# assafmu/wav2letter_pytorch

Hardware: AMD Instinct MI355X
Metric: audio-frames/sec/GPU (fwd+bwd+CTC), Wav2Letter 64-mel x 1000-frame bf16 (higher is better)
Workload: dtype bf16

## Files before the change

wav2letter_pytorch_amd/csrc/conv_igemm.hip:

```cpp
#include "common.h"
#include "../../include/w2l_hip.h"
#include <algorithm>
#include <array>
#include <map>
#include <vector>
#include <mutex>
#include <tuple>
#include <type_traits>
#include <utility>

namespace {

constexpr int BK = 64;
constexpr int ROWB = BK * 2;

struct IgemmParams {
    const bf16_raw* x;
    const bf16_raw* w;
    void* y;
    const float* bias;
    union { float* stats; uint8_t* fz_q; };
    int stats_slots;
    int64_t x_rows_per_utt;
    int64_t x_max_row;
    int N, Cin, Cout, Tout, Kw, stride, dil;
    int tiles_t, ncols, xrows_lds;
    int y_f32, accumulate;
    int splits;
    float* slabs;
    unsigned* tickets;
    int sk_ranges, sk_total;
    float descale;
    union { const float* descale_dev; unsigned long long* fz_clip; };
    union { const bf16_raw* bn_y; const bf16_raw* fz_res; };
    union { const float* bn_scale; const float* fz_scale; };
    union { const float* bn_shift; const float* fz_shift; };
    union { const float* bn_mean; const bf16_raw* fz_res_lo; };
    union { const float* bn_invstd; bf16_raw* fz_out; };
    union { const uint8_t* bn_mask; bf16_raw* fz_out_lo; };
    union { const int32_t* bn_lens; const int32_t* fz_lens; };
    union { int bn_T; int fz_rows; };
    union { int bn_pad_l; int fz_pad_l; };
    union { int bn_pad_mode; int fz_pad_mode; };
    union { int bn_per; int fz_pad_r; };
    int bn_Tp;
    union { int bn_act; int fz_act; };
    union { float bn_gk; float fz_qscale; };
};

typedef int v4i __attribute__((ext_vector_type(4)));
typedef int v8i __attribute__((ext_vector_type(8)));
__device__ __forceinline__ f32x4 mfma_e4m3_k128(bf16x8 a_lo, bf16x8 a_hi, bf16x8 b_lo, bf16x8 b_hi, f32x4 c) {
    const v4i al = __builtin_bit_cast(v4i, a_lo), ah = __builtin_bit_cast(v4i, a_hi);
    const v4i bl = __builtin_bit_cast(v4i, b_lo), bh = __builtin_bit_cast(v4i, b_hi);
    const v8i av = __builtin_shufflevector(al, ah, 0, 1, 2, 3, 4, 5, 6, 7);
    const v8i bv = __builtin_shufflevector(bl, bh, 0, 1, 2, 3, 4, 5, 6, 7);
    return __builtin_amdgcn_mfma_scale_f32_16x16x128_f8f6f4(av, bv, c, 0, 0, 0, 0x7f7f7f7f, 0, 0x7f7f7f7f);
}

__device__ __forceinline__ void glds16(const void* gsrc, void* lds_dst_wave_base) {
    __builtin_amdgcn_global_load_lds((const __attribute__((address_space(1))) void*)gsrc,
                                     (__attribute__((address_space(3))) void*)lds_dst_wave_base, 16, 0, 0);
}

template <int G> struct QVec { typedef unsigned type __attribute__((ext_vector_type(G))); };
template <> struct QVec<1> { typedef unsigned type; };

struct SkPiece { int tile, s_begin, s_end, nsplit, split; int64_t slab_base; };
__host__ __device__ inline SkPiece sk_piece(int W, int G, int S_, int r, int w_cur, int w_end) {
    SkPiece q;
    q.tile = w_cur / S_;
    q.s_begin = w_cur - q.tile * S_;
    q.s_end = q.s_begin + (w_end - w_cur) < S_ ? q.s_begin + (w_end - w_cur) : S_;
    const int r_lo = (int)((((int64_t)q.tile * S_ + 1) * G + W - 1) / W) - 1;
    const int r_hi = (int)((((int64_t)q.tile * S_ + S_) * G + W - 1) / W) - 1;
    q.nsplit = r_hi - r_lo + 1;
    q.split = r - r_lo;
    q.slab_base = (int64_t)r_lo + q.tile;
    return q;
}

template <int MW, int NW, int MS, int NS, int S, int PIPE, bool F8 = false, int EPI = 0, bool SK = false>
__global__ __launch_bounds__(64 * MW * NW, 2) void conv_igemm_kernel(IgemmParams p) {
    static_assert(!SK || (!F8 && EPI == 0 && S == 1), "stream-K is built for the plain bf16 stride-1 kernels");
    static_assert(!(F8 && PIPE != 0), "the e4m3 kernel is built for K-loop structure 0 only");
    static_assert(EPI != 1 || (!F8 && S == 1), "the fused BatchNorm-backward epilogue belongs to bf16 data gradients");
    constexpr int ESZ = F8 ? 1 : 2;
    constexpr int BKE = ROWB / ESZ;
    constexpr int BM = 16 * MW * MS, BN = 16 * NW * NS, NWAVES = MW * NW, NT = 64 * NWAVES;
    extern __shared__ __attribute__((aligned(1024))) char smem[];
    const int tid = threadIdx.x;
    const int lane = tid & 63;
    const int wave = __builtin_amdgcn_readfirstlane(tid >> 6);
    const int wm = wave / NW, wn = wave % NW;

    const int lin = xcd_remap(blockIdx.x, gridDim.x);
    int w_cur = 0, w_end = 0;
    if constexpr (SK) {
        w_cur = (int)(((int64_t)p.sk_total * lin) / p.sk_ranges);
        w_end = (int)(((int64_t)p.sk_total * (lin + 1)) / p.sk_ranges);
    }
    do {
    int split, tile, nsplit, sk_begin = 0, sk_end = 0;
    int64_t slab_base;
    if constexpr (SK) {
        __syncthreads();
        const SkPiece q = sk_piece(p.sk_total, p.sk_ranges, (p.Cin / (ROWB / (F8 ? 1 : 2))) * p.Kw, lin, w_cur, w_end);
        tile = q.tile;
        sk_begin = q.s_begin;
        sk_end = q.s_end;
        w_cur += sk_end - sk_begin;
        nsplit = q.nsplit;
        split = q.split;
        slab_base = q.slab_base;
    } else {
        nsplit = p.splits;
        split = nsplit > 1 ? lin % nsplit : 0;
        tile = nsplit > 1 ? lin / nsplit : lin;
        slab_base = (int64_t)tile * nsplit;
    }
    const int tm = tile / p.ncols;
    const int col = tile - tm * p.ncols;
    const int n = col / p.tiles_t;
    const int tt = col - n * p.tiles_t;
    const int m0 = tm * BM;
    const int t0 = tt * BN;

    constexpr int s = S;
    const int d = p.dil, Kw = p.Kw, Cin = p.Cin;
    const int xrows = p.xrows_lds;
    char* wbuf0 = smem;
    char* wbuf1 = smem + BM * ROWB;
    char* xbuf0 = smem + 2 * BM * ROWB;
    char* xbuf1 = xbuf0 + xrows * ROWB;

    const int64_t xrow0 = (int64_t)n * p.x_rows_per_utt + (int64_t)t0 * s;

    const int srow = lane >> 3;
    const int schunk = lane & 7;
    const int gchunk = schunk ^ srow;
    constexpr int WGROUPS = BM / 8;
    constexpr int W_PER_WAVE = (WGROUPS + NWAVES - 1) / NWAVES;
    unsigned w_voff[W_PER_WAVE];
#pragma unroll
    for (int i = 0; i < W_PER_WAVE; ++i) {
        int co = m0 + (wave + i * NWAVES) * 8 + srow;
        co = co < p.Cout ? co : p.Cout - 1;
        w_voff[i] = (unsigned)co * (unsigned)Cin * (unsigned)ESZ + (unsigned)gchunk * 16u;
    }
    const int64_t w_tap_bytes = (int64_t)p.Cout * Cin * ESZ;
    auto stage_w = [&](char* dst, int kw, int c) {
        W2L_DIAG_SKIP_DMA(p);
        const char* slab = reinterpret_cast<const char*>(p.w) + kw * w_tap_bytes + c * (BK * 2);
#pragma unroll
        for (int i = 0; i < W_PER_WAVE; ++i) {
            const int grp = wave + i * NWAVES;
            if ((WGROUPS % NWAVES == 0) || grp < WGROUPS) glds16(slab + w_voff[i], dst + grp * 1024);
        }
    };
    auto stage_x = [&](char* dst, int c) {
        W2L_DIAG_SKIP_DMA(p);
        const int ngrp = xrows >> 3;
        for (int grp = wave; grp < ngrp; grp += NWAVES) {
            int64_t r = xrow0 + grp * 8 + srow;
            r = r < p.x_max_row ? r : p.x_max_row;
            const char* src = reinterpret_cast<const char*>(p.x) + (r * Cin + (int64_t)c * BKE) * ESZ + gchunk * 16;
            glds16(src, dst + grp * 1024);
        }
    };

    f32x4 acc[MS][NS];
#pragma unroll
    for (int i = 0; i < MS; ++i)
#pragma unroll
        for (int j = 0; j < NS; ++j) acc[i][j] = f32x4{0.f, 0.f, 0.f, 0.f};

    const int nchunks = Cin / BKE;
    const int total_steps = nchunks * Kw;
    const int s_begin = SK ? sk_begin : (nsplit > 1 ? (int)(((int64_t)total_steps * split) / nsplit) : 0);
    const int s_end = SK ? sk_end : (nsplit > 1 ? (int)(((int64_t)total_steps * (split + 1)) / nsplit) : total_steps);
    const int nsteps = s_end - s_begin;
    const int c_first = s_begin / Kw, kw_first = s_begin - c_first * Kw;

    const int fr = lane & 15, fq = lane >> 4;
    constexpr int CH1_XOR = F8 ? 16 : 64;
    const int ch0 = F8 ? 2 * fq : fq;
    const int a_lane0 = (wm * MS * 16 + fr) * ROWB + ((ch0 ^ (fr & 7)) << 4);
    const int a_lane1 = a_lane0 ^ CH1_XOR;
    const int b_row0 = (wn * NS * 16 + fr) * s;

    if constexpr (PIPE == 0) {
        stage_x((c_first & 1) ? xbuf1 : xbuf0, c_first);
        stage_w(wbuf0, kw_first, c_first);

        int kw = kw_first, c = c_first;
        for (int step = 0; step < nsteps; ++step) {
            asm volatile("s_waitcnt vmcnt(0)" ::: "memory");
            __syncthreads();
            int kw_n = kw + 1, c_n = c;
            if (kw_n == Kw) { kw_n = 0; c_n = c + 1; }
            if (step + 1 < nsteps) {
                stage_w((step & 1) ? wbuf0 : wbuf1, kw_n, c_n);
                if (kw_n == 0) stage_x((c_n & 1) ? xbuf1 : xbuf0, c_n);
            }
            const char* wb = (step & 1) ? wbuf1 : wbuf0;
            const char* xb = (c & 1) ? xbuf1 : xbuf0;
            const char* A0 = wb + a_lane0;
            const char* A1 = wb + a_lane1;
            const int tsh = b_row0 + kw * d;
            const int sw0 = ((ch0 ^ (tsh & 7)) << 4);
            const char* Bb = xb + (tsh << 7);
            const char* B0 = Bb + sw0;
            const char* B1 = Bb + (sw0 ^ CH1_XOR);
            bf16x8 a0[MS], b0[NS], a1[MS], b1[NS];
    #pragma unroll
// ... 189 lines not shown
                    const bool ok = co_ok[g] && t < Tout;
                    f32x4 v = acc[mi0 + g][ni] * descale + bias4[g];
                    v = v * sc4[g] + sh4[g];
                    if (p.fz_res && ok) {
                        const u16x4 rv = *reinterpret_cast<const u16x4*>(p.fz_res + ((int64_t)n * Tout + t) * Cout + co);
#pragma unroll
                        for (int r = 0; r < 4; ++r) v[r] += bf16_bits_to_f32(rv[r]);
                    }
                    u16x4 hi;
                    float a[4];
#pragma unroll
                    for (int r = 0; r < 4; ++r) {
                        a[r] = v[r];
                        if (p.fz_act == 1) a[r] = fminf(fmaxf(a[r], 0.f), 20.f);
                        else if (p.fz_act == 2) a[r] = fmaxf(a[r], 0.f);
                        if (t >= len_n) a[r] = 0.f;
                        hi[r] = f32_to_bf16_bits(a[r]);
                        if (ok && fabsf(a[r]) > q_limit) ++clipped;
                        a[r] = fminf(fmaxf(a[r] * qs, -448.f), 448.f);
                    }
                    int w = __builtin_amdgcn_cvt_pk_fp8_f32(a[0], a[1], 0, false);
                    w = __builtin_amdgcn_cvt_pk_fp8_f32(a[2], a[3], w, true);
                    q[g] = (unsigned)w;
                    if (obase && ok) {
                        put(pl + t, co, hi);
                        if (p.fz_pad_mode == 1) {
                            if (t >= 1 && t <= pl) put(pl - t, co, hi);
                            const int j = Tout - 1 - t;
                            if (j >= 1 && j <= pr) put(pl + Tout - 1 + j, co, hi);
                        }
                    }
                    if (obase && p.fz_pad_mode != 1 && tt == 0 && co_ok[g]) {
                        const u16x4 z = u16x4{0, 0, 0, 0};
                        if (tl < pl) put(tl, co, z);
                        if (tl < pr) put(pl + Tout + tl, co, z);
                    }
                }
#pragma unroll
                for (int b = 1; b < G; b <<= 1) {
                    const bool up = (fq & b) != 0;
#pragma unroll
                    for (int i = 0; i < G; ++i) {
                        if (i & b) continue;
                        const unsigned send = up ? q[i] : q[i | b];
                        const unsigned recv = (unsigned)__shfl_xor((int)send, 16 * b, 64);
                        if (up) q[i] = recv; else q[i | b] = recv;
                    }
                }
                if (qbase) {
                    qvec qv = {}, z = {};
                    if constexpr (G == 1) {
                        qv = q[0];
                    } else {
#pragma unroll
                        for (int g = 0; g < G; ++g) qv[g] = q[g];
                    }
                    if (coq_ok && t < Tout) {
                        putq(pl + t, qv);
                        if (p.fz_pad_mode == 1) {
                            if (t >= 1 && t <= pl) putq(pl - t, qv);
                            const int j = Tout - 1 - t;
                            if (j >= 1 && j <= pr) putq(pl + Tout - 1 + j, qv);
                        }
                    }
                    if (p.fz_pad_mode != 1 && tt == 0 && coq_ok) {
                        if (tl < pl) putq(tl, z);
                        if (tl < pr) putq(pl + Tout + tl, z);
                    }
                }
            }
        };
#pragma unroll
        for (int g4 = 0; g4 < MS / 4; ++g4) group(std::integral_constant<int, 4>{}, g4 * 4);
        if constexpr ((MS & 3) >= 2) group(std::integral_constant<int, 2>{}, (MS / 4) * 4);
        if constexpr (MS & 1) group(std::integral_constant<int, 1>{}, MS - 1);
        if (p.fz_clip) {
#pragma unroll
            for (int m = 1; m < 64; m <<= 1) clipped += __shfl_xor(clipped, m, 64);
            __syncthreads();
            unsigned* red = reinterpret_cast<unsigned*>(smem);
            if (lane == 0) red[wave] = clipped;
            __syncthreads();
            if (tid == 0) {
                unsigned total = 0;
                for (int w = 0; w < NWAVES; ++w) total += red[w];
                if (total) atomicAdd(p.fz_clip, (unsigned long long)total);
            }
        }
    } else if constexpr (EPI == 2) {
        const int pl = p.fz_pad_l, pr = p.fz_pad_r;
        const int len_n = p.fz_lens ? p.fz_lens[n] : Tout;
        bf16_raw* const obase = p.fz_out + (int64_t)n * p.fz_rows * Cout;
        bf16_raw* const obase_lo = p.fz_out_lo ? p.fz_out_lo + (int64_t)n * p.fz_rows * Cout : nullptr;
        auto put = [&](int row, int co, u16x4 hi, u16x4 lo) {
            const int64_t o = (int64_t)row * Cout + co;
            *reinterpret_cast<u16x4*>(obase + o) = hi;
            if (obase_lo) *reinterpret_cast<u16x4*>(obase_lo + o) = lo;
        };
#pragma unroll
        for (int mi = 0; mi < MS; ++mi) {
            const int co = m0 + (wm * MS + mi) * 16 + fq * 4;
            const bool co_ok = co < Cout;
            f32x4 bias4 = f32x4{0.f, 0.f, 0.f, 0.f}, sc4 = f32x4{1.f, 1.f, 1.f, 1.f}, sh4 = bias4;
            if (p.bias && co_ok) bias4 = *reinterpret_cast<const f32x4*>(p.bias + co);
            if (p.fz_scale && co_ok) {
                sc4 = *reinterpret_cast<const f32x4*>(p.fz_scale + co);
                sh4 = *reinterpret_cast<const f32x4*>(p.fz_shift + co);
            }
#pragma unroll
            for (int ni = 0; ni < NS; ++ni) {
                const int tl = (wn * NS + ni) * 16 + fr;
                const int t = t0 + tl;
                const bool ok = co_ok && t < Tout;
                if (ok) {
                    const int64_t off = ((int64_t)n * Tout + t) * Cout + co;
                    f32x4 v = acc[mi][ni] + bias4;
                    if (p.accumulate) v += *reinterpret_cast<const f32x4*>(reinterpret_cast<const float*>(p.y) + off);
                    v = v * sc4 + sh4;
                    if (p.fz_res) {
                        const u16x4 rv = *reinterpret_cast<const u16x4*>(p.fz_res + off);
#pragma unroll
                        for (int r = 0; r < 4; ++r) v[r] += bf16_bits_to_f32(rv[r]);
                        if (p.fz_res_lo) {
                            const u16x4 rl = *reinterpret_cast<const u16x4*>(p.fz_res_lo + off);
#pragma unroll
                            for (int r = 0; r < 4; ++r) v[r] += bf16_bits_to_f32(rl[r]);
                        }
                    }
                    u16x4 hi, lo = u16x4{0, 0, 0, 0};
#pragma unroll
                    for (int r = 0; r < 4; ++r) {
                        float a = v[r];
                        if (p.fz_act == 1) a = fminf(fmaxf(a, 0.f), 20.f);
                        else if (p.fz_act == 2) a = fmaxf(a, 0.f);
                        if (t >= len_n) a = 0.f;
                        hi[r] = f32_to_bf16_bits(a);
                        if (obase_lo) lo[r] = f32_to_bf16_bits(a - bf16_bits_to_f32(hi[r]));
                    }
                    put(pl + t, co, hi, lo);
                    if (p.fz_pad_mode == 1) {
                        if (t >= 1 && t <= pl) put(pl - t, co, hi, lo);
                        const int j = Tout - 1 - t;
                        if (j >= 1 && j <= pr) put(pl + Tout - 1 + j, co, hi, lo);
                    }
                }
                if (p.fz_pad_mode != 1 && tt == 0 && co_ok) {
                    const u16x4 z = u16x4{0, 0, 0, 0};
                    if (tl < pl) put(tl, co, z, z);
                    if (tl < pr) put(pl + Tout + tl, co, z, z);
                }
            }
        }
    } else {
    float s1[MS][4], s2[MS][4];
#pragma unroll
    for (int mi = 0; mi < MS; ++mi) {
        const int co = m0 + (wm * MS + mi) * 16 + fq * 4;
        const bool co_ok = co < Cout;
        f32x4 bias4 = f32x4{0.f, 0.f, 0.f, 0.f};
        if (p.bias && co_ok) bias4 = *reinterpret_cast<const f32x4*>(p.bias + co);
#pragma unroll
        for (int r = 0; r < 4; ++r) { s1[mi][r] = 0.f; s2[mi][r] = 0.f; }
#pragma unroll
        for (int ni = 0; ni < NS; ++ni) {
            const int t = t0 + (wn * NS + ni) * 16 + fr;
            const bool ok = co_ok && t < Tout;
            f32x4 v = F8 ? acc[mi][ni] * descale + bias4 : acc[mi][ni] + bias4;
            const int64_t off = ((int64_t)n * Tout + t) * Cout + co;
            if (ok) {
                if (p.y_f32) {
                    float* yp = reinterpret_cast<float*>(p.y) + off;
                    if (p.accumulate) v += *reinterpret_cast<const f32x4*>(yp);
                    *reinterpret_cast<f32x4*>(yp) = v;
                } else {
                    u16x4 o;
#pragma unroll
                    for (int r = 0; r < 4; ++r) o[r] = f32_to_bf16_bits(v[r]);
                    *reinterpret_cast<u16x4*>(reinterpret_cast<bf16_raw*>(p.y) + off) = o;
                }
                if constexpr (EPI == 0) {
#pragma unroll
                    for (int r = 0; r < 4; ++r) { s1[mi][r] += v[r]; s2[mi][r] += v[r] * v[r]; }
                }
            }
        }
    }
    if constexpr (EPI == 1) {
        int64_t yrow[NS];
        bool live[NS];
#pragma unroll
        for (int ni = 0; ni < NS; ++ni) {
            const int t = t0 + (wn * NS + ni) * 16 + fr;
            const int tc = t < Tout ? t : Tout - 1;
            const int nu = (int)((unsigned)tc / (unsigned)p.bn_per);
            const int u = tc - nu * p.bn_per;
            int ts = u - p.bn_pad_l;
            bool lv = t < Tout && u < p.bn_Tp;
            if (ts < 0 || ts >= p.bn_T) {
                if (p.bn_pad_mode == 1) ts = ts < 0 ? -ts : 2 * (p.bn_T - 1) - ts;
                else lv = false;
            }
            ts = ts < 0 ? 0 : (ts >= p.bn_T ? p.bn_T - 1 : ts);
            if (lv && p.bn_lens && ts >= p.bn_lens[nu]) lv = false;
            live[ni] = lv;
            yrow[ni] = (int64_t)nu * p.bn_T + ts;
        }
        constexpr int CH = MS % 4 == 0 ? 4 : (MS % 2 == 0 ? 2 : 1);
        __syncthreads();
        float* red = reinterpret_cast<float*>(smem);
#pragma unroll
        for (int m0i = 0; m0i < MS; m0i += CH) {
            u16x4 yv[CH][NS];
            unsigned mb[CH][NS];
#pragma unroll
            for (int c = 0; c < CH; ++c) {
                int co = m0 + (wm * MS + m0i + c) * 16 + fq * 4;
                co = co < Cout ? co : Cout - 4;
#pragma unroll
                for (int ni = 0; ni < NS; ++ni) {
                    yv[c][ni] = *reinterpret_cast<const u16x4*>(p.bn_y + yrow[ni] * Cout + co);
                    mb[c][ni] = p.bn_mask ? (unsigned)p.bn_mask[yrow[ni] * (Cout >> 3) + (co >> 3)] : 0xFFu;
                }
            }
#pragma unroll
            for (int c = 0; c < CH; ++c) {
                const int mi = m0i + c;
                const int co = m0 + (wm * MS + mi) * 16 + fq * 4;
                const bool co_ok = co < Cout;
                const int cc = co_ok ? co : Cout - 4;
                f32x4 bsc = f32x4{1.f, 1.f, 1.f, 1.f}, bsh = f32x4{0.f, 0.f, 0.f, 0.f}, bmu = bsh, bis = bsh;
                if (p.bn_scale) { bsc = *reinterpret_cast<const f32x4*>(p.bn_scale + cc); bsh = *reinterpret_cast<const f32x4*>(p.bn_shift + cc); }
                if (p.bn_mean) { bmu = *reinterpret_cast<const f32x4*>(p.bn_mean + cc); bis = *reinterpret_cast<const f32x4*>(p.bn_invstd + cc); }
#pragma unroll
                for (int ni = 0; ni < NS; ++ni) {
                    const bool on = live[ni] && co_ok;
                    const unsigned bits = mb[c][ni] >> (co & 4);
#pragma unroll
                    for (int r = 0; r < 4; ++r) {
                        const float yf = bf16_bits_to_f32(yv[c][ni][r]);
                        const bool keep = (bits >> r) & 1u;
                        float z = yf * bsc[r] + bsh[r];
                        z = keep ? z * p.bn_gk : 0.f;
                        bool pass = keep && on;
                        if (p.bn_act == 1) pass = pass && z >= 0.f && z <= 20.f;
                        else if (p.bn_act == 2) pass = pass && z > 0.f;
                        const float g = pass ? acc[mi][ni][r] * p.bn_gk : 0.f;
                        s1[mi][r] += g;
                        s2[mi][r] += g * ((yf - bmu[r]) * bis[r]);
                    }
                }
#pragma unroll
                for (int r = 0; r < 4; ++r) {
                    float a = s1[mi][r], b = s2[mi][r];
#pragma unroll
                    for (int m = 1; m < 16; m <<= 1) {
                        a += __shfl_xor(a, m, 64);
                        b += __shfl_xor(b, m, 64);
                    }
                    if (fr == 0) {
                        const int cl = (wm * MS + mi) * 16 + fq * 4 + r;
                        red[(wn * 2 + 0) * BM + cl] = a;
                        red[(wn * 2 + 1) * BM + cl] = b;
                    }
                }
            }
        }
    }
    if (p.stats) {
        constexpr int HALVES = BN / 128;
        constexpr int WPH = NW / HALVES;
        static_assert(BN % 128 == 0 || true, "");
        float* red = reinterpret_cast<float*>(smem);
        if constexpr (EPI == 0) {
            __syncthreads();
#pragma unroll
            for (int mi = 0; mi < MS; ++mi)
#pragma unroll
                for (int r = 0; r < 4; ++r) {
                    float a = s1[mi][r], b = s2[mi][r];
#pragma unroll
                    for (int m = 1; m < 16; m <<= 1) {
                        a += __shfl_xor(a, m, 64);
                        b += __shfl_xor(b, m, 64);
                    }
                    if (fr == 0) {
                        const int cl = (wm * MS + mi) * 16 + fq * 4 + r;
                        red[(wn * 2 + 0) * BM + cl] = a;
                        red[(wn * 2 + 1) * BM + cl] = b;
                    }
                }
        }
        __syncthreads();
        if (p.stats_slots) {
            float* dst = p.stats + (((int64_t)n * p.tiles_t + tt) % p.stats_slots) * 2 * Cout;
            for (int cl = tid; cl < BM; cl += NT) {
                if (m0 + cl < Cout) {
                    float a = 0.f, b = 0.f;
#pragma unroll
                    for (int w = 0; w < NW; ++w) {
                        a += red[(w * 2 + 0) * BM + cl];
                        b += red[(w * 2 + 1) * BM + cl];
                    }
                    atomicAdd(dst + m0 + cl, a);
                    atomicAdd(dst + Cout + m0 + cl, b);
                }
            }
        } else {
        const int tiles128 = (Tout + 127) / 128;
        for (int idx = tid; idx < BM * HALVES; idx += NT) {
            const int h = idx / BM, cl = idx - h * BM;
            const int trow = tt * HALVES + h;
            if (m0 + cl < Cout && trow < tiles128) {
                float a = 0.f, b = 0.f;
#pragma unroll
                for (int w = 0; w < WPH; ++w) {
                    a += red[((h * WPH + w) * 2 + 0) * BM + cl];
                    b += red[((h * WPH + w) * 2 + 1) * BM + cl];
                }
                const int64_t srow = (int64_t)n * tiles128 + trow;
                float* dst = p.stats + srow * 2 * Cout;
                dst[m0 + cl] = a;
                dst[Cout + m0 + cl] = b;
            }
        }
        }
    }
    }
    } while (SK && w_cur < w_end);
}

struct TileCfg { int mw, nw, ms, ns; float eff; };
constexpr TileCfg kCfgs[] = {
    {2, 2, 2, 4, 0.83f}, {2, 2, 3, 4, 1.00f}, {2, 2, 4, 4, 1.00f}, {2, 2, 5, 4, 1.01f},
    {4, 2, 3, 4, 0.90f}, {4, 2, 4, 4, 0.92f},
    {2, 3, 2, 3, 0.80f}, {2, 3, 3, 3, 0.97f}, {2, 3, 4, 3, 0.97f}, {2, 3, 5, 3, 0.98f},
    {2, 4, 2, 4, 0.85f}, {2, 4, 3, 4, 0.97f}, {2, 4, 4, 4, 1.00f}, {2, 4, 5, 4, 1.04f},
    {2, 4, 6, 4, 1.10f}, {2, 4, 7, 4, 1.06f}, {2, 4, 8, 4, 1.12f},
    {2, 3, 4, 6, 1.00f}, {2, 3, 5, 6, 1.00f}, {2, 3, 6, 6, 1.00f}, {2, 3, 7, 6, 1.00f},
    {2, 4, 4, 6, 1.00f}, {2, 4, 5, 6, 1.00f}, {2, 4, 6, 6, 1.00f},
    {2, 4, 4, 7, 1.00f}, {2, 4, 5, 7, 1.00f},
};
constexpr int kNumCfgs = sizeof(kCfgs) / sizeof(kCfgs[0]);
constexpr int kSpillCfg = 20;

constexpr size_t kLdsBytes = 160 * 1024;
constexpr int kCUs = 256;
constexpr size_t kTicketBytes = 64 * 1024;
constexpr int kFzMaxPad = 96;
constexpr int kWaveCap = 16, kSkWaveCap = 8;

struct ConvProblem {
    const void* x;
    int64_t x_bstride, x_rows_total;
    const void* w;
    void* y;
    int y_f32, accumulate;
    const float* bias;
    float* stats;
    int N, Cin, Cout, Tout, Kw, stride, dil;
    void* ws;
    int64_t ws_bytes;
    hipStream_t stream;
    bool f8 = false;
    float descale = 1.f;
    const float* descale_dev = nullptr;
    int stats_slots = 0;
};

enum EpiKind { kEpiNone = 0, kEpiBnReduce, kEpiInfer, kEpiInferF8 };
struct Epilogue {
    EpiKind kind;
    struct { const w2l_bnact_t* d; int pad_l, pad_r, pad_mode, per; } bn;
    const w2l_bnact_epi_t* fz;
    void* out_q;
    float q_scale;
    int64_t* q_clipped;
};
constexpr Epilogue kNoEpilogue{};
static inline bool is_infer(const Epilogue* ep) { return ep->kind == kEpiInfer || ep->kind == kEpiInferF8; }

static int stats_flag(const ConvProblem& pr, const Epilogue* ep) {
    if (is_infer(ep)) return 3;
    return pr.stats == nullptr ? 0 : (!pr.f8 && pr.stats_slots > 0 ? 2 : 1);
}

struct TileGeom {
    int bm, bn, xrows, waves, tiles_m, tiles_t;
    size_t lds;
    int64_t blocks;
};
static TileGeom tile_geom(const TileCfg& c, const ConvProblem& pr) {
    TileGeom g;
    g.bm = 16 * c.mw * c.ms;
    g.bn = 16 * c.nw * c.ns;
    g.xrows = ((g.bn - 1) * pr.stride + (pr.Kw - 1) * pr.dil + 1 + 7) & ~7;
    g.waves = c.mw * c.nw;
    g.tiles_m = (pr.Cout + g.bm - 1) / g.bm;
    g.tiles_t = (pr.Tout + g.bn - 1) / g.bn;
    g.lds = 2 * (size_t)g.bm * ROWB + 2 * (size_t)g.xrows * ROWB;
    g.blocks = (int64_t)g.tiles_m * pr.N * g.tiles_t;
    return g;
}
static ConvProblem window_only(int Kw, int stride, int dil) {
    ConvProblem pr{};
    pr.Kw = Kw; pr.stride = stride; pr.dil = dil;
    return pr;
}
static int blocks_per_cu(const TileGeom& g, int wave_cap) {
    const int by_lds = (int)(kLdsBytes / g.lds), by_waves = wave_cap / g.waves;
    const int per_cu = by_lds < by_waves ? by_lds : by_waves;
    return per_cu < 1 ? 1 : per_cu;
}
static double last_round_fill(int64_t blocks, int64_t slots) {
// ... 65 lines not shown

template <int MW, int NW, int MS, int NS>
int launch_f8(const ConvPlan& pl) {
    if (pl.epi == 2) {
        if constexpr (f8_fused_built(NW, MS, NS)) {
            return launch_kernel(conv_igemm_kernel<MW, NW, MS, NS, 1, 0, true, 2>, pl);
        } else {
            w2l_set_error("conv1d_igemm_bnact_fp8: block shape not built for the fused epilogue");
            return 1;
        }
    }
    return launch_kernel(conv_igemm_kernel<MW, NW, MS, NS, 1, 0, true>, pl);
}

typedef int (*LaunchFn)(const ConvPlan&);
template <int I> constexpr LaunchFn kLaunchCfg = &launch_cfg<kCfgs[I].mw, kCfgs[I].nw, kCfgs[I].ms, kCfgs[I].ns>;
template <int I> constexpr LaunchFn kLaunchF8 = &launch_f8<kCfgs[I].mw, kCfgs[I].nw, kCfgs[I].ms, kCfgs[I].ns>;
template <size_t... I>
constexpr std::array<LaunchFn, sizeof...(I)> cfg_launchers(std::index_sequence<I...>) { return {{kLaunchCfg<(int)I>...}}; }
template <size_t... K>
constexpr std::array<LaunchFn, sizeof...(K)> f8_launchers(std::index_sequence<K...>) { return {{kLaunchF8<kF8Cfgs[K]>...}}; }
constexpr auto kCfgLaunchers = cfg_launchers(std::make_index_sequence<kNumCfgs>{});
constexpr auto kF8Launchers = f8_launchers(std::make_index_sequence<kNumF8Cfgs>{});

int launch(const ConvPlan& pl) { return (pl.f8 ? kF8Launchers[pl.idx] : kCfgLaunchers[pl.shape])(pl); }

}

constexpr int kSplits[] = {1, 2, 3, 4, 5, 6, 8, 0};
constexpr int kNumSplits = sizeof(kSplits) / sizeof(kSplits[0]);
constexpr int kMaxSplit = 8;
constexpr int kSkMinSteps = 8;
constexpr int kBaseCfgs = 2 * kNumCfgs;
static thread_local int g_force_cfg = -1;
static thread_local int g_force_f8 = -1;
static thread_local int g_stats_slots = 0;
extern "C" void w2l_conv_stats_mode(int slots) { g_stats_slots = slots < 0 ? 0 : (slots > 64 ? 64 : slots); }
extern "C" void w2l_conv_force_tile_config(int idx) { g_force_cfg = idx; }
extern "C" void w2l_conv_force_fp8_config(int idx) { g_force_f8 = idx; }
W2L_DIAG_IGEMM_EXPORTS

typedef std::tuple<int, int, int, int, int, int, int, int> ShapeKey;
static std::map<ShapeKey, int> g_tuned, g_tuned_f8;
static std::mutex g_tuned_mu;
static ShapeKey shape_key(const ConvProblem& pr, int sflag) {
    return ShapeKey(pr.N, pr.Cin, pr.Cout, pr.Tout, pr.Kw, pr.stride, pr.dil, sflag);
}

static bool cfg_feasible(int idx, const ConvProblem& pr, int sflag) {
    if (idx < 0 || idx >= kBaseCfgs * kNumSplits) return false;
    const int i = idx % kNumCfgs;
    const TileGeom g = tile_geom(kCfgs[i], pr);
    if (sflag == 1 && !bn128_ok(g)) return false;
    if (pr.stride != 1 && i != 2) return false;
    if (i == kSpillCfg) return false;
    return g.lds <= kLdsBytes;
}

static bool f8_feasible(int k, const ConvProblem& pr, int sflag) {
    if (k < 0 || k >= kNumF8Cfgs) return false;
    const TileCfg& c = kCfgs[kF8Cfgs[k]];
    const TileGeom g = tile_geom(c, pr);
    if (sflag == 3 && (!f8_fused_built(c.nw, c.ms, c.ns) || g.bn <= kFzMaxPad)) return false;
    if (sflag == 1 && !bn128_ok(g)) return false;
    return g.lds <= kLdsBytes;
}

static int choose_cfg(const ConvProblem& pr, int sflag, int forced) {
    if (forced >= 0) return (pr.f8 ? f8_feasible(forced, pr, sflag) : cfg_feasible(forced, pr, sflag)) ? forced : -1;
    {
        std::lock_guard<std::mutex> lock(g_tuned_mu);
        const auto& tuned = pr.f8 ? g_tuned_f8 : g_tuned;
        auto it = tuned.find(shape_key(pr, sflag));
        if (it != tuned.end()) return it->second;
    }
    int best = -1;
    double best_cost = 1e30;
    for (int k = 0; k < (pr.f8 ? kNumF8Cfgs : kNumCfgs); ++k) {
        if (!(pr.f8 ? f8_feasible(k, pr, sflag) : cfg_feasible(k, pr, sflag))) continue;
        const TileCfg& c = kCfgs[pr.f8 ? kF8Cfgs[k] : k];
        const double cost = tile_cost(tile_geom(c, pr), c.eff, pr.f8 ? 1.0 : 0.75, k);
        if (cost < best_cost) { best_cost = cost; best = k; }
    }
    return best;
}

extern "C" int w2l_conv_stat_tiles(int N, int Tout) { return N * ((Tout + 127) / 128); }

static size_t splitk_bytes(const TileGeom& g, int splits) {
    return kTicketBytes + (size_t)g.blocks * splits * g.bm * g.bn * sizeof(float);
}

static int sk_ranges(const TileGeom& g) { return kCUs * blocks_per_cu(g, kSkWaveCap); }

static bool sk_feasible(const TileGeom& g, const ConvProblem& pr) {
    if (pr.ws == nullptr || pr.stride != 1) return false;
    const int64_t tiles = g.blocks, steps = (int64_t)(pr.Cin / BK) * pr.Kw, G = sk_ranges(g);
    if (tiles * steps / G < kSkMinSteps || (tiles * steps + steps) * G >= (1LL << 31)) return false;
    return tiles * (int64_t)sizeof(unsigned) <= (int64_t)kTicketBytes &&
           (int64_t)kTicketBytes + (tiles + G) * g.bm * g.bn * (int64_t)sizeof(float) <= pr.ws_bytes;
}

static bool split_feasible(const TileGeom& g, int splits, const ConvProblem& pr) {
    if (splits == 1) return true;
    if (pr.ws == nullptr || (pr.Cin / BK) * pr.Kw < 2 * splits) return false;
    return (size_t)g.blocks * sizeof(unsigned) <= kTicketBytes && splitk_bytes(g, splits) <= (size_t)pr.ws_bytes;
}

static int check_infer_epi(const w2l_bnact_epi_t* e, int Tout, const char* who) {
    W2L_CHECK_ARG(e->pad_l >= 0 && e->pad_r >= 0 && e->pad_l <= kFzMaxPad && e->pad_r <= kFzMaxPad &&
                  e->out_rows >= e->pad_l + Tout + e->pad_r,
                  "%s: bad output geometry (pads %d,%d of at most %d; %d rows for %d frames)", who, e->pad_l, e->pad_r,
                  kFzMaxPad, e->out_rows, Tout);
    W2L_CHECK_ARG(e->pad_mode != 1 || (e->pad_l < Tout && e->pad_r < Tout), "%s: reflect pad (%d,%d) needs pad < T=%d", who,
                  e->pad_l, e->pad_r, Tout);
    W2L_CHECK_ARG((e->scale == nullptr) == (e->shift == nullptr) && e->act >= 0 && e->act <= 2 && (e->res || !e->res_lo),
                  "%s: scale/shift come together, act is 0..2, res_lo needs res", who);
    return 0;
}

static int plan(const ConvProblem& pr, const Epilogue* ep, int forced, ConvPlan& pl) {
    const char* who = pr.f8 ? "conv1d_igemm_fp8" : "conv1d_igemm";
    W2L_CHECK_ARG(pr.x && pr.w && (pr.y || is_infer(ep)), "%s: null pointer", who);
    W2L_CHECK_ARG(pr.f8 ? ep->kind == kEpiNone || ep->kind == kEpiInferF8 : ep->kind != kEpiInferF8,
                  "%s: epilogue of the other operand type", who);
    W2L_CHECK_ARG(pr.N > 0 && pr.Tout > 0 && pr.Kw > 0 && (pr.stride == 1 || (pr.stride == 2 && !pr.f8)) && pr.dil > 0,
                  "%s: bad sizes (stride must be 1 or 2; e4m3: 1)", who);
    const int cin_unit = pr.f8 ? 128 : 64;
    W2L_CHECK_ARG(pr.Cin % cin_unit == 0 && pr.Cin > 0, "%s: Cin=%d must be a positive multiple of %d", who, pr.Cin, cin_unit);
    W2L_CHECK_ARG(pr.Cout % 64 == 0 && pr.Cout > 0, "%s: Cout=%d must be a positive multiple of 64", who, pr.Cout);
    W2L_CHECK_ARG(pr.x_bstride % pr.Cin == 0, "%s: x_bstride must be a multiple of Cin", who);
    W2L_CHECK_ARG(!(pr.accumulate && !pr.y_f32), "%s: accumulate needs fp32 output", who);
    W2L_CHECK_ARG(pr.descale > 0.f, "%s: descale must be positive", who);
    IgemmParams& p = pl.p;
    p.x = (const bf16_raw*)pr.x;
    p.w = (const bf16_raw*)pr.w;
    p.y = pr.y;
    p.bias = pr.bias;
    p.stats = pr.stats;
    p.stats_slots = pr.stats ? pr.stats_slots : 0;
    p.x_rows_per_utt = pr.x_bstride / pr.Cin;
    p.x_max_row = pr.x_rows_total - 1;
    p.N = pr.N; p.Cin = pr.Cin; p.Cout = pr.Cout; p.Tout = pr.Tout; p.Kw = pr.Kw; p.stride = pr.stride; p.dil = pr.dil;
    p.y_f32 = pr.y_f32; p.accumulate = pr.accumulate;
    p.descale = pr.descale;
    p.descale_dev = pr.descale_dev;
    pl.epi = 0;
    if (ep->kind == kEpiBnReduce) {
        const w2l_bnact_t* d = ep->bn.d;
        const int pad_l = ep->bn.pad_l, pad_r = ep->bn.pad_r, per = ep->bn.per;
        W2L_CHECK_ARG(d && d->y && !d->y_f32 && !d->y2 && pr.stats && !pr.y_f32 && !pr.accumulate && !pr.bias && pr.N == 1 &&
                      pr.stride == 1,
                      "conv1d_dgrad_bnreduce: needs a bf16 single-branch layer, a statistics buffer and a flat bf16 output");
        W2L_CHECK_ARG(d->C == pr.Cout && per > 0 && pad_l >= 0 && pad_r >= 0 && (int64_t)d->N * per <= pr.Tout &&
                      per >= pad_l + d->T + pad_r,
                      "conv1d_dgrad_bnreduce: geometry mismatch (C=%d vs %d, per=%d, N=%d, rows=%d)", d->C, pr.Cout, per, d->N,
                      pr.Tout);
        W2L_CHECK_ARG(d->drop_p == 0.f || d->mask, "conv1d_dgrad_bnreduce: dropout needs the recorded mask");
        p.bn_y = (const bf16_raw*)d->y;
        p.bn_scale = d->scale; p.bn_shift = d->shift; p.bn_mean = d->mean; p.bn_invstd = d->invstd;
        p.bn_mask = d->drop_p > 0.f ? d->mask : nullptr;
        p.bn_lens = d->lens;
        p.bn_T = d->T; p.bn_pad_l = pad_l; p.bn_pad_mode = ep->bn.pad_mode; p.bn_per = per;
        p.bn_Tp = pad_l + d->T + pad_r;
        p.bn_act = d->act;
        p.bn_gk = d->drop_p > 0.f ? 1.f / (1.f - d->drop_p) : 1.f;
        pl.epi = 1;
    } else if (is_infer(ep)) {
        const w2l_bnact_epi_t* e = ep->fz;
        const bool q = ep->kind == kEpiInferF8 && ep->out_q != nullptr;
        const char* who_fz = pr.f8 ? "conv1d_igemm_bnact_fp8" : "conv1d_igemm_bnact";
        if (pr.f8) {
            W2L_CHECK_ARG(e && (e->out_hi || q) && !e->out_lo && !e->res_lo && !pr.y && !pr.stats && !pr.descale_dev,
                          "conv1d_igemm_bnact_fp8: needs an e4m3 or a bf16 output and takes no lo halves");
            W2L_CHECK_ARG(!q || (ep->q_scale > 0.f && ((uintptr_t)ep->out_q & 15) == 0),
                          "conv1d_igemm_bnact_fp8: the e4m3 output needs a positive scale and 16-byte alignment");
        } else {
            W2L_CHECK_ARG(e && pr.stats == nullptr && e->out_hi, "conv1d_igemm_bnact: null output / bad combination");
        }
        if (int rc = check_infer_epi(e, pr.Tout, who_fz)) return rc;
        p.stats_slots = 0;
        p.fz_q = q ? (uint8_t*)ep->out_q : nullptr;
        p.fz_qscale = q ? ep->q_scale : 1.f;
        p.fz_clip = q ? (unsigned long long*)ep->q_clipped : nullptr;
        p.fz_scale = e->scale; p.fz_shift = e->shift;
        p.fz_res = (const bf16_raw*)e->res; p.fz_res_lo = (const bf16_raw*)e->res_lo;
        p.fz_lens = e->lens;
        p.fz_out = (bf16_raw*)e->out_hi; p.fz_out_lo = (bf16_raw*)e->out_lo;
        p.fz_rows = e->out_rows; p.fz_pad_l = e->pad_l; p.fz_pad_r = e->pad_r; p.fz_pad_mode = e->pad_mode;
        p.fz_act = e->act;
        pl.epi = 2;
    }
    const int64_t need = (int64_t)(pr.N - 1) * p.x_rows_per_utt + (int64_t)(pr.Tout - 1) * pr.stride + (int64_t)(pr.Kw - 1) * pr.dil;
    W2L_CHECK_ARG(need <= p.x_max_row, "%s: padded input too small (need row %lld, have %lld)", who, (long long)need,
                  (long long)p.x_max_row);
    pl.idx = choose_cfg(pr, stats_flag(pr, ep), forced);
    W2L_CHECK_ARG(pl.idx >= 0, "%s: no block shape fits LDS (Kw=%d dil=%d stride=%d)", who, pr.Kw, pr.dil, pr.stride);
    pl.f8 = pr.f8;
    pl.shape = pr.f8 ? kF8Cfgs[pl.idx] : pl.idx % kNumCfgs;
    pl.pipe = pr.f8 ? 0 : (pl.idx % kBaseCfgs) / kNumCfgs;
    const TileCfg& c = kCfgs[pl.shape];
    const TileGeom g = tile_geom(c, pr);
    p.tiles_t = g.tiles_t;
    p.ncols = pr.N * g.tiles_t;
    p.xrows_lds = g.xrows;
    int splits = pr.f8 ? 1 : kSplits[pl.idx / kBaseCfgs];
    p.sk_ranges = 0;
    p.sk_total = 0;
    if (splits == 0) {
        if (pl.epi == 0 && sk_feasible(g, pr)) {
            p.sk_ranges = sk_ranges(g);
            p.sk_total = g.tiles_m * p.ncols * ((pr.Cin / BK) * pr.Kw);
        }
        splits = 1;
    }
    if (!split_feasible(g, splits, pr)) splits = 1;
    p.splits = splits;
    p.tickets = (unsigned*)pr.ws;
    p.slabs = pr.ws ? (float*)((char*)pr.ws + kTicketBytes) : nullptr;
    pl.splits = splits;
    pl.sk_ranges = p.sk_ranges;
    pl.grid = p.sk_ranges > 0 ? (unsigned)p.sk_ranges : (unsigned)(g.tiles_m * splits * p.ncols);
    pl.threads = 64 * g.waves;
    pl.lds = g.lds;
    pl.stream = pr.stream;
    return 0;
}

struct EventPair {
    hipEvent_t e0 = nullptr, e1 = nullptr;
    ~EventPair() {
        if (e0) (void)hipEventDestroy(e0);
        if (e1) (void)hipEventDestroy(e1);
    }
};

template <typename MakePlan>
static float time_candidate(const MakePlan& make, int n, const EventPair& ev) {
    ConvPlan pl;
    if (make(pl) != 0 || launch(pl) != 0) return -1.f;
    (void)hipEventRecord(ev.e0, pl.stream);
    for (int r = 0; r < n; ++r) launch(pl);
    (void)hipEventRecord(ev.e1, pl.stream);
    if (hipEventSynchronize(ev.e1) != hipSuccess) return -1.f;
    float ms = 0.f;
    if (hipEventElapsedTime(&ms, ev.e0, ev.e1) != hipSuccess) return -1.f;
    return ms;
}

static int tune(const ConvProblem& pr, const Epilogue* ep, int reps) {
    const int sflag = stats_flag(pr, ep);
    const ShapeKey key = shape_key(pr, sflag);
    auto& table = pr.f8 ? g_tuned_f8 : g_tuned;
    {
        std::lock_guard<std::mutex> lock(g_tuned_mu);
        if (table.count(key)) return 0;
    }
    EventPair ev;
    W2L_CHECK_HIP(hipEventCreate(&ev.e0));
    W2L_CHECK_HIP(hipEventCreate(&ev.e1));
    if (reps < 1) reps = 1;
    if (pr.ws) (void)hipMemsetAsync(pr.ws, 0, kTicketBytes, pr.stream);
    auto time_cfg = [&](int i, int n) -> float {
        float ms = time_candidate([&](ConvPlan& pl) { return plan(pr, ep, i, pl); }, n, ev);
        if (!pr.f8 && kSplits[i / kBaseCfgs] == 0) ms *= 1.03f;
        return ms;
    };
    int best = -1;
    if (pr.f8) {
        float best_ms = 1e30f;
        for (int k = 0; k < kNumF8Cfgs; ++k) {
            if (!f8_feasible(k, pr, sflag)) continue;
            const float ms = time_cfg(k, reps);
            if (ms >= 0.f && ms < best_ms) { best_ms = ms; best = k; }
        }
    } else {
        std::vector<std::pair<float, int>> timed;
        for (int i = 0; i < kBaseCfgs * kNumSplits; ++i) {
            if (!cfg_feasible(i, pr, sflag)) continue;
            const int splits = kSplits[i / kBaseCfgs];
            const TileGeom g = tile_geom(kCfgs[i % kNumCfgs], pr);
            if (splits == 0) {
                if (ep->kind != kEpiNone || !sk_feasible(g, pr)) continue;
                const int64_t slots = sk_ranges(g);
                if (last_round_fill(g.blocks, slots) > 0.85 || g.blocks > 4 * slots) continue;
            } else if (splits > 1) {
                if (!split_feasible(g, splits, pr)) continue;
                const int64_t slots = (int64_t)kCUs * blocks_per_cu(g, kWaveCap);
                if (last_round_fill(g.blocks, slots) > 0.92 || g.blocks * splits > 6 * slots ||
                    (pr.Cin / BK) * pr.Kw / splits < 8)
                    continue;
            }
            const float ms = time_cfg(i, reps);
            if (ms >= 0.f) timed.emplace_back(ms, i);
        }
        std::sort(timed.begin(), timed.end());
        best = timed.empty() ? -1 : timed[0].second;
        const int finalists = timed.size() < kFinalists ? (int)timed.size() : kFinalists;
        if (finalists > 1) {
            float total[kFinalists] = {};
            for (int round = 0; round < kFinalRounds; ++round)
                for (int k = 0; k < finalists; ++k) {
                    const float ms = time_cfg(timed[k].second, 4 * reps);
                    total[k] += ms >= 0.f ? ms : 1e30f;
                }
            int kb = 0;
            for (int k = 1; k < finalists; ++k)
                if (total[k] < total[kb]) kb = k;
            best = timed[kb].second;
        }
    }
    W2L_CHECK_ARG(best >= 0, "%s_tune: no feasible block shape", pr.f8 ? "conv1d_igemm_fp8" : "conv1d_igemm");
    std::lock_guard<std::mutex> lock(g_tuned_mu);
    table[key] = best;
    return 0;
}

static int run(ConvProblem pr, const Epilogue* ep, int reps = 0) {
    pr.stats_slots = pr.stats ? g_stats_slots : 0;
    if (reps != 0) return tune(pr, ep, reps);
    ConvPlan pl;
    if (int rc = plan(pr, ep, pr.f8 ? g_force_f8 : g_force_cfg, pl)) return rc;
    return launch(pl);
}

extern "C" int w2l_conv1d_igemm_ws(const void* xp, int64_t x_bstride, int64_t x_rows_total, const void* w, void* y,
                                   int y_f32, int accumulate, const float* bias, float* stats_partial, int N, int Cin,
                                   int Cout, int Tout, int Kw, int stride, int dil, void* splitk_ws, int64_t splitk_ws_bytes,
                                   void* stream) {
    return run({xp, x_bstride, x_rows_total, w, y, y_f32, accumulate, bias, stats_partial, N, Cin, Cout, Tout, Kw, stride, dil,
                splitk_ws, splitk_ws_bytes, (hipStream_t)stream}, &kNoEpilogue);
}

extern "C" int w2l_conv1d_dgrad_bnreduce_ws(const void* dy, int64_t dy_rows_total, const void* w_dgr, void* dxp, float* partial,
                                            const w2l_bnact_t* d, int pad_l, int pad_r, int pad_mode, int per, int Cconv_out,
                                            int flat_rows, int Kw, int dil, void* splitk_ws, int64_t splitk_ws_bytes,
                                            void* stream) {
    W2L_CHECK_ARG(d != nullptr, "conv1d_dgrad_bnreduce: null descriptor");
    const Epilogue ep{kEpiBnReduce, {d, pad_l, pad_r, pad_mode, per}};
    return run({dy, dy_rows_total * Cconv_out, dy_rows_total, w_dgr, dxp, 0, 0, nullptr, partial, 1, Cconv_out, d->C, flat_rows,
                Kw, 1, dil, splitk_ws, splitk_ws_bytes, (hipStream_t)stream}, &ep);
}

extern "C" int w2l_conv1d_igemm(const void* xp, int64_t x_bstride, int64_t x_rows_total, const void* w, void* y,
                                int y_f32, int accumulate, const float* bias, float* stats_partial, int N, int Cin,
                                int Cout, int Tout, int Kw, int stride, int dil, void* stream) {
    return w2l_conv1d_igemm_ws(xp, x_bstride, x_rows_total, w, y, y_f32, accumulate, bias, stats_partial, N, Cin, Cout, Tout,
                               Kw, stride, dil, nullptr, 0, stream);
}

extern "C" int w2l_conv1d_igemm_bnact_ws(const void* xp, int64_t x_bstride, int64_t x_rows_total, const void* w,
                                         const float* acc_in, const float* bias, const w2l_bnact_epi_t* e, int N, int Cin,
                                         int Cout, int Tout, int Kw, int stride, int dil, void* splitk_ws,
                                         int64_t splitk_ws_bytes, void* stream) {
    W2L_CHECK_ARG(e != nullptr, "conv1d_igemm_bnact: null descriptor");
    const Epilogue ep{kEpiInfer, {}, e};
    return run({xp, x_bstride, x_rows_total, w, (void*)acc_in, 1, acc_in != nullptr, bias, nullptr, N, Cin, Cout, Tout, Kw,
                stride, dil, splitk_ws, splitk_ws_bytes, (hipStream_t)stream}, &ep);
// ... 171 lines not shown
```

Baseline: 2.552 million.

## Stage BN-reduce epilogue operands into LDS via async global-to-LDS loads

In the dgrad+BN-reduce epilogue, the per-row gather indices are computed once per tile by one thread per row and kept in a shared table. The activation slice, the dropout mask and the per-channel BN constants are then brought into LDS with async global_load_lds copies, possibly in several passes, instead of scattered per-thread global loads. This aims to replace uncoalesced row-gather reads with coalesced staged transfers and to cut redundant index math. In exchange it adds barriers and LDS footprint, and it tightens the geometry check to require N*per == Tout.

Result: no change. 2.549 million (median of 2 runs) (-0.1%).

```diff
diff --git a/wav2letter_pytorch_amd/csrc/conv_igemm.hip b/wav2letter_pytorch_amd/csrc/conv_igemm.hip
--- a/wav2letter_pytorch_amd/csrc/conv_igemm.hip
+++ b/wav2letter_pytorch_amd/csrc/conv_igemm.hip
@@ -61,6 +61,11 @@
 __device__ __forceinline__ void glds16(const void* gsrc, void* lds_dst_wave_base) {
     __builtin_amdgcn_global_load_lds((const __attribute__((address_space(1))) void*)gsrc,
                                      (__attribute__((address_space(3))) void*)lds_dst_wave_base, 16, 0, 0);
+}
+
+__device__ __forceinline__ void glds4(const void* gsrc, void* lds_dst_wave_base) {
+    __builtin_amdgcn_global_load_lds((const __attribute__((address_space(1))) void*)gsrc,
+                                     (__attribute__((address_space(3))) void*)lds_dst_wave_base, 4, 0, 0);
 }
 
 template <int G> struct QVec { typedef unsigned type __attribute__((ext_vector_type(G))); };
@@ -556,13 +561,124 @@
             }
         }
     } else {
+    constexpr int EP_RED = NW * 2 * BM * 4;
+    constexpr int EP_J = BM / 32;
+    constexpr int EP_MINSTR = (EP_J * BN + 63) / 64;
+    constexpr int EP_P = (MW * MS + 3) / 4;
+    constexpr int EP_YG = (BN / 8 + NWAVES - 1) / NWAVES;
+    constexpr int EP_PINSTR = 4 * BM / 64;
+    constexpr int EP_PG = (EP_PINSTR + NWAVES - 1) / NWAVES;
+    constexpr int EP_MG = (EP_MINSTR + NWAVES - 1) / NWAVES;
+    static_assert(EPI != 1 || (BN <= NT && BN % 16 == 0 && BM % 32 == 0), "one thread per tile row forms the row table");
+    int* const ep_rowtab = reinterpret_cast<int*>(smem + EP_RED);
+    float* const ep_ptab = reinterpret_cast<float*>(smem + EP_RED + BN * 4);
+    unsigned* const ep_mtab = reinterpret_cast<unsigned*>(smem + EP_RED + BN * 4 + 16 * BM);
+    const int ep_yoff = (EP_RED + BN * 4 + 16 * BM + (p.bn_mask ? EP_MINSTR * 256 : 0) + 1023) & ~1023;
+    char* const ep_ybuf = smem + ep_yoff;
+    const int ep_fit = ((2 * BM + 2 * xrows) * ROWB - ep_yoff) / (BN * ROWB);
+    const int ep_pp = ep_fit < EP_P ? ep_fit : EP_P;
+    const int ep_mp = ep_pp * 4 / MW;
+    auto ep_y_rows = [&](int* yr) {
+#pragma unroll
+        for (int i = 0; i < EP_YG; ++i) {
+            const int grp = wave + i * NWAVES;
+            yr[i] = ep_rowtab[(grp < BN / 8 ? grp : 0) * 8 + srow] & 0x7fffffff;
+        }
+    };
+    auto ep_issue_y = [&](int mi0, const int* yr) {
+        unsigned choff[EP_P];
+#pragma unroll
+        for (int pn = 0; pn < EP_P; ++pn) {
+            const int st = pn * 4 + (gchunk >> 1);
+            const int wq = (st >= ep_mp) + (st >= 2 * ep_mp) + (st >= 3 * ep_mp);
+            int mq = mi0 + st - wq * ep_mp;
+            mq = mq < MS ? mq : MS - 1;
+            int ch = m0 + (wq * MS + mq) * 16 + (gchunk & 1) * 8;
+            ch = ch < p.Cout ? ch : p.Cout - 8;
+            choff[pn] = (unsigned)ch * 2u;
+        }
+#pragma unroll
+        for (int i = 0; i < EP_YG; ++i) {
+            const int grp = wave + i * NWAVES;
+            if (((BN / 8) % NWAVES == 0) || grp < BN / 8) {
+                const char* rbase = reinterpret_cast<const char*>(p.bn_y) + (int64_t)yr[i] * p.Cout * 2;
+#pragma unroll
+                for (int pn = 0; pn < EP_P; ++pn)
+                    if (pn < ep_pp) glds16(rbase + choff[pn], ep_ybuf + pn * (BN * ROWB) + grp * 1024);
+            }
+        }
+    };
+    auto ep_mask_src = [&](const uint8_t** src) {
+        const int cb = p.Cout >> 3;
+#pragma unroll
+        for (int i = 0; i < EP_MG; ++i) {
+            const int k = wave + i * NWAVES;
+            const int slot = (k < EP_MINSTR ? k : 0) * 64 + lane;
+            int j = slot / BN;
+            const int row = slot - j * BN;
+            j = j < EP_J ? j : EP_J - 1;
+            int c32 = m0 + 32 * j;
+            c32 = c32 < p.Cout ? c32 : p.Cout - 32;
+            src[i] = p.bn_mask + (int64_t)(ep_rowtab[row] & 0x7fffffff) * cb + (c32 >> 3);
+        }
+    };
+    auto ep_issue_consts = [&]() {
+#pragma unroll
+        for (int i = 0; i < EP_PG; ++i) {
+            const int k = wave + i * NWAVES;
+            const int slot = k * 64 + lane;
+            const int a = slot / BM;
+            int c = m0 + slot - a * BM;
+            c = c < p.Cout ? c : p.Cout - 1;
+            const float* arr = a == 0 ? p.bn_scale : (a == 1 ? p.bn_shift : (a == 2 ? p.bn_mean : p.bn_invstd));
+            const float* src = arr ? arr + c : reinterpret_cast<const float*>(p.bn_y);
+            if ((EP_PINSTR % NWAVES == 0) || k < EP_PINSTR) glds4(src, ep_ptab + k * 64);
+        }
+    };
+    auto ep_issue_mask = [&](const uint8_t* const* src) {
+#pragma unroll
+        for (int i = 0; i < EP_MG; ++i) {
+            const int k = wave + i * NWAVES;
+            if ((EP_MINSTR % NWAVES == 0) || k < EP_MINSTR) glds4(src[i], ep_mtab + k * 64);
+        }
+    };
+    unsigned ep_live = 0;
+    if constexpr (EPI == 1) {
+        __syncthreads();
+        if (tid < BN) {
+            const int t = t0 + tid;
+            const int tc = t < p.Tout ? t : p.Tout - 1;
+            const int nu = (int)((unsigned)tc / (unsigned)p.bn_per);
+            const int u = tc - nu * p.bn_per;
+            int ts = u - p.bn_pad_l;
+            bool lv = t < p.Tout && u < p.bn_Tp;
+            if (ts < 0 || ts >= p.bn_T) {
+                if (p.bn_pad_mode == 1) ts = ts < 0 ? -ts : 2 * (p.bn_T - 1) - ts;
+                else lv = false;
+            }
+            ts = ts < 0 ? 0 : (ts >= p.bn_T ? p.bn_T - 1 : ts);
+            if (lv && p.bn_lens && ts >= p.bn_lens[nu]) lv = false;
+            ep_rowtab[tid] = (nu * p.bn_T + ts) | (lv ? 0 : (int)0x80000000);
+        }
+        __syncthreads();
+#pragma unroll
+        for (int ni = 0; ni < NS; ++ni)
+            if (ep_rowtab[(wn * NS + ni) * 16 + fr] >= 0) ep_live |= 1u << ni;
+        int yr[EP_YG];
+        const uint8_t* msrc[EP_MG];
+        ep_y_rows(yr);
+        if (p.bn_mask) ep_mask_src(msrc);
+        ep_issue_y(0, yr);
+        if (p.bn_mask) ep_issue_mask(msrc);
+        ep_issue_consts();
+    }
     float s1[MS][4], s2[MS][4];
 #pragma unroll
     for (int mi = 0; mi < MS; ++mi) {
         const int co = m0 + (wm * MS + mi) * 16 + fq * 4;
         const bool co_ok = co < Cout;
         f32x4 bias4 = f32x4{0.f, 0.f, 0.f, 0.f};
-        if (p.bias && co_ok) bias4 = *reinterpret_cast<const f32x4*>(p.bias + co);
+        if (EPI != 1 && p.bias && co_ok) bias4 = *reinterpret_cast<const f32x4*>(p.bias + co);
 #pragma unroll
         for (int r = 0; r < 4; ++r) { s1[mi][r] = 0.f; s2[mi][r] = 0.f; }
 #pragma unroll
@@ -572,7 +688,7 @@
             f32x4 v = F8 ? acc[mi][ni] * descale + bias4 : acc[mi][ni] + bias4;
             const int64_t off = ((int64_t)n * Tout + t) * Cout + co;
             if (ok) {
-                if (p.y_f32) {
+                if (EPI != 1 && p.y_f32) {
                     float* yp = reinterpret_cast<float*>(p.y) + off;
                     if (p.accumulate) v += *reinterpret_cast<const f32x4*>(yp);
                     *reinterpret_cast<f32x4*>(yp) = v;
@@ -590,58 +706,46 @@
         }
     }
     if constexpr (EPI == 1) {
-        int64_t yrow[NS];
-        bool live[NS];
-#pragma unroll
-        for (int ni = 0; ni < NS; ++ni) {
-            const int t = t0 + (wn * NS + ni) * 16 + fr;
-            const int tc = t < Tout ? t : Tout - 1;
-            const int nu = (int)((unsigned)tc / (unsigned)p.bn_per);
-            const int u = tc - nu * p.bn_per;
-            int ts = u - p.bn_pad_l;
-            bool lv = t < Tout && u < p.bn_Tp;
-            if (ts < 0 || ts >= p.bn_T) {
-                if (p.bn_pad_mode == 1) ts = ts < 0 ? -ts : 2 * (p.bn_T - 1) - ts;
-                else lv = false;
-            }
-            ts = ts < 0 ? 0 : (ts >= p.bn_T ? p.bn_T - 1 : ts);
-            if (lv && p.bn_lens && ts >= p.bn_lens[nu]) lv = false;
-            live[ni] = lv;
-            yrow[ni] = (int64_t)nu * p.bn_T + ts;
-        }
-        constexpr int CH = MS % 4 == 0 ? 4 : (MS % 2 == 0 ? 2 : 1);
-        __syncthreads();
         float* red = reinterpret_cast<float*>(smem);
-#pragma unroll
-        for (int m0i = 0; m0i < MS; m0i += CH) {
-            u16x4 yv[CH][NS];
-            unsigned mb[CH][NS];
-#pragma unroll
-            for (int c = 0; c < CH; ++c) {
-                int co = m0 + (wm * MS + m0i + c) * 16 + fq * 4;
-                co = co < Cout ? co : Cout - 4;
+        for (int mi0 = 0; mi0 < MS; mi0 += ep_mp) {
+            if (mi0 > 0) {
+                __syncthreads();
+                int yr[EP_YG];
+                ep_y_rows(yr);
+                ep_issue_y(mi0, yr);
+            }
+            asm volatile("s_waitcnt vmcnt(0)" ::: "memory");
+            __syncthreads();
+#pragma unroll
+            for (int mi = 0; mi < MS; ++mi) {
+                if (mi < mi0 || mi >= mi0 + ep_mp) continue;
+                const int st = wm * ep_mp + (mi - mi0);
+                const char* yb = ep_ybuf + (st >> 2) * (BN * ROWB) + (wn * NS * 16 + fr) * ROWB +
+                                 (((((st & 3) << 1) | (fq >> 1)) ^ (fr & 7)) << 4) + ((fq & 1) << 3);
+                const int q = wm * MS + mi;
+                const unsigned* mbp = ep_mtab + (q >> 1) * BN + wn * NS * 16 + fr;
+                const int bitpos = ((q & 1) << 4) + (fq << 2);
+                u16x4 yv[NS];
+                unsigned mb[NS];
 #pragma unroll
                 for (int ni = 0; ni < NS; ++ni) {
-                    yv[c][ni] = *reinterpret_cast<const u16x4*>(p.bn_y + yrow[ni] * Cout + co);
-                    mb[c][ni] = p.bn_mask ? (unsigned)p.bn_mask[yrow[ni] * (Cout >> 3) + (co >> 3)] : 0xFFu;
+                    yv[ni] = *reinterpret_cast<const u16x4*>(yb + ni * 16 * ROWB);
+                    mb[ni] = p.bn_mask ? mbp[ni * 16] >> bitpos : 0xFu;
                 }
-            }
-#pragma unroll
-            for (int c = 0; c < CH; ++c) {
-                const int mi = m0i + c;
-                const int co = m0 + (wm * MS + mi) * 16 + fq * 4;
+                const int co = m0 + q * 16 + fq * 4;
                 const bool co_ok = co < Cout;
-                const int cc = co_ok ? co : Cout - 4;
+                const float* pt = ep_ptab + q * 16 + fq * 4;
                 f32x4 bsc = f32x4{1.f, 1.f, 1.f, 1.f}, bsh = f32x4{0.f, 0.f, 0.f, 0.f}, bmu = bsh, bis = bsh;
-                if (p.bn_scale) { bsc = *reinterpret_cast<const f32x4*>(p.bn_scale + cc); bsh = *reinterpret_cast<const f32x4*>(p.bn_shift + cc); }
-                if (p.bn_mean) { bmu = *reinterpret_cast<const f32x4*>(p.bn_mean + cc); bis = *reinterpret_cast<const f32x4*>(p.bn_invstd + cc); }
+                if (p.bn_scale) { bsc = *reinterpret_cast<const f32x4*>(pt); bsh = *reinterpret_cast<const f32x4*>(pt + BM); }
+                if (p.bn_mean) { bmu = *reinterpret_cast<const f32x4*>(pt + 2 * BM); bis = *reinterpret_cast<const f32x4*>(pt + 3 * BM); }
+                float a1[4] = {0.f, 0.f, 0.f, 0.f}, a2[4] = {0.f, 0.f, 0.f, 0.f};
 #pragma unroll
                 for (int ni = 0; ni < NS; ++ni) {
-                    const bool on = live[ni] && co_ok;
-                    const unsigned bits = mb[c][ni] >> (co & 4);
+                    const bool on = ((ep_live >> ni) & 1u) && co_ok;
+                    const unsigned bits = mb[ni];
 #pragma unroll
                     for (int r = 0; r < 4; ++r) {
-                        const float yf = bf16_bits_to_f32(yv[c][ni][r]);
+                        const float yf = bf16_bits_to_f32(yv[ni][r]);
                         const bool keep = (bits >> r) & 1u;
                         float z = yf * bsc[r] + bsh[r];
                         z = keep ? z * p.bn_gk : 0.f;
@@ -649,20 +753,20 @@
                         if (p.bn_act == 1) pass = pass && z >= 0.f && z <= 20.f;
                         else if (p.bn_act == 2) pass = pass && z > 0.f;
                         const float g = pass ? acc[mi][ni][r] * p.bn_gk : 0.f;
-                        s1[mi][r] += g;
-                        s2[mi][r] += g * ((yf - bmu[r]) * bis[r]);
+                        a1[r] += g;
+                        a2[r] += g * ((yf - bmu[r]) * bis[r]);
                     }
                 }
 #pragma unroll
                 for (int r = 0; r < 4; ++r) {
-                    float a = s1[mi][r], b = s2[mi][r];
+                    float a = a1[r], b = a2[r];
 #pragma unroll
                     for (int m = 1; m < 16; m <<= 1) {
                         a += __shfl_xor(a, m, 64);
                         b += __shfl_xor(b, m, 64);
                     }
                     if (fr == 0) {
-                        const int cl = (wm * MS + mi) * 16 + fq * 4 + r;
+                        const int cl = q * 16 + fq * 4 + r;
                         red[(wn * 2 + 0) * BM + cl] = a;
                         red[(wn * 2 + 1) * BM + cl] = b;
                     }
@@ -1034,7 +1138,7 @@
         W2L_CHECK_ARG(d && d->y && !d->y_f32 && !d->y2 && pr.stats && !pr.y_f32 && !pr.accumulate && !pr.bias && pr.N == 1 &&
                       pr.stride == 1,
                       "conv1d_dgrad_bnreduce: needs a bf16 single-branch layer, a statistics buffer and a flat bf16 output");
-        W2L_CHECK_ARG(d->C == pr.Cout && per > 0 && pad_l >= 0 && pad_r >= 0 && (int64_t)d->N * per <= pr.Tout &&
+        W2L_CHECK_ARG(d->C == pr.Cout && per > 0 && pad_l >= 0 && pad_r >= 0 && (int64_t)d->N * per == pr.Tout &&
                       per >= pad_l + d->T + pad_r,
                       "conv1d_dgrad_bnreduce: geometry mismatch (C=%d vs %d, per=%d, N=%d, rows=%d)", d->C, pr.Cout, per, d->N,
                       pr.Tout);
@@ -1086,6 +1190,12 @@
     p.tiles_t = g.tiles_t;
     p.ncols = pr.N * g.tiles_t;
     p.xrows_lds = g.xrows;
+    if (pl.epi == 1) {
+        const size_t mask_bytes = p.bn_mask ? ((size_t)(g.bm / 32) * g.bn + 63) / 64 * 256 : 0;
+        const size_t head = ((size_t)c.nw * 2 * g.bm * 4 + (size_t)g.bn * 4 + (size_t)16 * g.bm + mask_bytes + 1023) & ~(size_t)1023;
+        W2L_CHECK_ARG(head + (size_t)g.bn * ROWB <= g.lds, "conv1d_dgrad_bnreduce: block shape %d leaves no LDS for the staged slice",
+                      pl.shape);
+    }
     int splits = pr.f8 ? 1 : kSplits[pl.idx / kBaseCfgs];
     p.sk_ranges = 0;
     p.sk_total = 0;
```
